# Dylan-H-Wang/skin-sm3

Measured on AMD Instinct MI355X. Metric: SM3 pretrain images/sec (paired 224x224), higher is better.
Workload: dtype bf16

## Files before the change

### skin-sm3_amd/csrc/conv_wgrad.hip

```cpp
#include <stdlib.h>

#include <atomic>

#include "conv_common.h"

namespace {

struct WgradParams {
    const char* x;
    const char* dy;
    float* dw;
    int M, Hi, Wi, Ci, Co;
    int sy, sx, ntaps;
    int dyt[SM3_MAX_TAPS], dxt[SM3_MAX_TAPS], wtap[SM3_MAX_TAPS];
    int w_row_stride;
    int HoWo, Wo, Ho;
    int adv_n, adv_oy, adv_ox;
    FastDiv div_HoWo, div_Wo;
    int tilesCo, tilesCi;
    int k_per_split;
    int gx, splits;
    uint32_t x_bytes;
    const char* dy1;
    float* dw1;
    int Co1, views, Mv, splits_view;
    long dw_view_stride, dw1_view_stride;
    long slab_stride;
    int slab_cap;
    float* dw_direct;
    int pair_rule, rmw;
    long g_x_bytes, g_dy_bytes, g_dw;
    int groups, x_ld, dy_ld;
};

#ifdef SM3_STAMP
__device__ unsigned long long* g_wstamp_buf = nullptr;
__device__ long g_wstamp_cap = 0;
#define SM3_WSTAMP_NOW() __builtin_amdgcn_s_memtime()
#endif

using sm3conv::dma16;
using sm3conv::dma_drain;
using sm3conv::kOOB;

template <int ROW_BYTES, bool BF16>
__device__ __forceinline__ uint32_t swz_bytes(int row) {
    if constexpr (!BF16) return 0u;
    else if constexpr (ROW_BYTES >= 256) return (uint32_t)(row & 3) << 6;
    else return (uint32_t)((row >> 1) & 1) << 6;
}

template <typename T, int BMW, int BNW, int KP, bool DENSE, int NST, int KG = 1, bool GRP = false>
__global__ __launch_bounds__(256 * KG, NST == 1 ? 4 : 1) void conv_wgrad_kernel(const WgradParams p) {
    static_assert(!GRP || DENSE, "grouped launches: the dense (1x1) loader");
    constexpr int SZ = sizeof(T);
    constexpr bool kBf16 = (SZ == 2);
    constexpr int RA = BMW * SZ, RB = BNW * SZ;
    constexpr int A_BYTES = KP * RA, B_BYTES = KP * RB, STAGE = A_BYTES + B_BYTES;
    constexpr int RPI_A = 1024 / RA, RPI_B = 1024 / RB;
    constexpr int AI = A_BYTES / 4096, BI = B_BYTES / 4096;
    constexpr int WTM = BMW / 2, WTN = BNW / 2, TM = WTM / 32, TN = WTN / 32;
    static_assert(AI >= 1 && BI >= 1 && TM >= 1 && TN >= 1 && RA <= 512 && RB <= 512, "unsupported tile");

    extern __shared__ __attribute__((aligned(16))) char smem[];
    const int tid = threadIdx.x, lane = tid & 63;
    const int wave_all = __builtin_amdgcn_readfirstlane(tid >> 6);
    const int wave = wave_all & 3, grp = wave_all >> 2;
#ifdef SM3_STAMP
    const unsigned long long st_entry = SM3_WSTAMP_NOW(), st_rentry = __builtin_amdgcn_s_memrealtime();
    unsigned long long st_seg[4] = {0, 0, 0, 0}, st_loop0 = 0, st_loop1 = 0;
#endif
    const int wm = wave >> 1, wn = wave & 1;

    int bx, slice;
    if (p.splits >= 8) {
        const int xcd = blockIdx.x & 7, q = blockIdx.x >> 3;
        bx = q % p.gx;
        slice = (q / p.gx) * 8 + xcd;
    } else {
        bx = blockIdx.x % p.gx;
        slice = blockIdx.x / p.gx;
    }
    if (slice >= p.splits) return;
    const int tci = bx % p.tilesCi;
    bx /= p.tilesCi;
    const int tap = bx % p.ntaps;
    const int tco = bx / p.ntaps;
    const int ci0 = tci * BNW;
    const bool second = tco * BMW >= p.Co;
    const int co0 = second ? tco * BMW - p.Co : tco * BMW;
    const int dyC = second ? p.Co1 : p.Co;
    const long gid = GRP ? (long)blockIdx.y : 0;
    const char* const dy_base = (second ? p.dy1 : p.dy) + (GRP ? gid * p.g_dy_bytes : 0);
    const char* const x_base = GRP ? p.x + gid * p.g_x_bytes : p.x;
    const int dyP = GRP ? p.dy_ld : dyC;
    const int xP = GRP ? p.x_ld : p.Ci;
    const int view = slice / p.splits_view;
    const int kbeg0 = view * p.Mv + (slice - view * p.splits_view) * p.k_per_split;
    const int kend = min((view + 1) * p.Mv, kbeg0 + p.k_per_split);
    if (kbeg0 >= kend) return;
    const int nsteps = ((kend - kbeg0 + KP - 1) / KP + KG - 1) / KG;
    const int kbeg = kbeg0 + grp * nsteps * KP;
    const int ddy = p.dyt[tap], ddx = p.dxt[tap];

    const __amdgpu_buffer_rsrc_t rdy =
        __builtin_amdgcn_make_buffer_rsrc((void*)dy_base, 0, (uint32_t)kend * (uint32_t)(dyP * SZ), 0x00020000);
    const __amdgpu_buffer_rsrc_t rx = __builtin_amdgcn_make_buffer_rsrc(
        (void*)x_base, 0, DENSE ? (uint32_t)kend * (uint32_t)(xP * SZ) : p.x_bytes, 0x00020000);

    const int a_rin = (lane * 16) / RA, a_pos = ((lane * 16) % RA) / 16;
    const int b_rin = (lane * 16) / RB, b_pos = ((lane * 16) % RB) / 16;
    uint32_t a_off[AI], b_off[BI];
    int b_row[BI];
    uint32_t b_cho[BI];
#pragma unroll
    for (int i = 0; i < AI; ++i) {
        const int r = (wave + 4 * i) * RPI_A + a_rin;
        const uint32_t lchunk = ((uint32_t)a_pos * 16u) ^ swz_bytes<RA, kBf16>(r);
        const bool col_ok = co0 + (int)(lchunk / SZ) < dyC;
        a_off[i] = col_ok ? (uint32_t)(kbeg + r) * (uint32_t)(dyP * SZ) + (uint32_t)(co0 * SZ) + lchunk : kOOB;
    }
#pragma unroll
    for (int i = 0; i < BI; ++i) {
        const int r = (wave + 4 * i) * RPI_B + b_rin;
        const uint32_t lchunk = ((uint32_t)b_pos * 16u) ^ swz_bytes<RB, kBf16>(r);
        const bool col_ok = ci0 + (int)(lchunk / SZ) < p.Ci;
        b_row[i] = col_ok ? r : -(1 << 28);
        b_cho[i] = (uint32_t)(ci0 * SZ) + lchunk;
        b_off[i] = col_ok ? (uint32_t)(kbeg + r) * (uint32_t)(xP * SZ) + b_cho[i] : kOOB;
    }
    const uint32_t smem_lds = (uint32_t)(uintptr_t)((__attribute__((address_space(3))) char*)smem);
    int g_m[BI], g_n[BI], g_oy[BI], g_ox[BI];
#pragma unroll
    for (int i = 0; i < BI; ++i) {
        g_m[i] = kbeg + b_row[i];
        const int m = g_m[i] < 0 ? 0 : g_m[i];
        g_n[i] = fdiv(m, p.div_HoWo);
        const int rem = m - g_n[i] * p.HoWo;
        g_oy[i] = fdiv(rem, p.div_Wo);
        g_ox[i] = rem - g_oy[i] * p.Wo;
    }

    auto dma_stage = [&](int stage, int step) {
        const uint32_t sA = smem_lds + (uint32_t)((grp * NST + stage) * STAGE) + (uint32_t)wave * 1024u;
        const uint32_t sB = sA + A_BYTES;
        const uint32_t soff_a = (uint32_t)(step * KP) * (uint32_t)(dyP * SZ);
#pragma unroll
        for (int i = 0; i < AI; ++i) dma16(rdy, sA + i * 4096, a_off[i], soff_a);
        if constexpr (DENSE) {
            const uint32_t soff_b = (uint32_t)(step * KP) * (uint32_t)(xP * SZ);
#pragma unroll
            for (int i = 0; i < BI; ++i) dma16(rx, sB + i * 4096, b_off[i], soff_b);
        } else {
#pragma unroll
            for (int i = 0; i < BI; ++i) {
                uint32_t off = kOOB;
                if (g_m[i] >= 0 && g_m[i] < kend) {
                    const int iy = g_oy[i] * p.sy + ddy, ix = g_ox[i] * p.sx + ddx;
                    if ((unsigned)iy < (unsigned)p.Hi && (unsigned)ix < (unsigned)p.Wi)
                        off = (uint32_t)((g_n[i] * p.Hi + iy) * p.Wi + ix) * (uint32_t)(p.Ci * SZ) + b_cho[i];
                }
                dma16(rx, sB + i * 4096, off, 0u);
                g_m[i] += KP;
                g_n[i] += p.adv_n;
                g_oy[i] += p.adv_oy;
                g_ox[i] += p.adv_ox;
                if (g_ox[i] >= p.Wo) {
                    g_ox[i] -= p.Wo;
                    ++g_oy[i];
                }
                if (g_oy[i] >= p.Ho) {
                    g_oy[i] -= p.Ho;
                    ++g_n[i];
                }
            }
        }
    };

    f32x16 acc[TM][TN];
#pragma unroll
    for (int i = 0; i < TM; ++i)
#pragma unroll
        for (int j = 0; j < TN; ++j)
#pragma unroll
            for (int r = 0; r < 16; ++r) acc[i][j][r] = 0.f;

    uint32_t ra_off[TM], rb_off[TN];
    if constexpr (kBf16) {
        const int g = lane >> 4, ii = lane & 15, q = ii >> 2, pq = ii & 3, h = g >> 1;
        const int colsel = 16 * (g & 1) + 4 * pq;
        const int krow0 = 8 * h + q;
#pragma unroll
        for (int i = 0; i < TM; ++i)
            ra_off[i] = (uint32_t)krow0 * RA + (((uint32_t)(wm * WTM + i * 32 + colsel) * 2u) ^ swz_bytes<RA, true>(q));
#pragma unroll
        for (int j = 0; j < TN; ++j)
            rb_off[j] = A_BYTES + (uint32_t)krow0 * RB + (((uint32_t)(wn * WTN + j * 32 + colsel) * 2u) ^ swz_bytes<RB, true>(q));
    } else {
        const int r = lane & 31, h = lane >> 5;
#pragma unroll
        for (int i = 0; i < TM; ++i) ra_off[i] = (uint32_t)h * RA + (uint32_t)(wm * WTM + i * 32 + r) * 4u;
#pragma unroll
        for (int j = 0; j < TN; ++j) rb_off[j] = A_BYTES + (uint32_t)h * RB + (uint32_t)(wn * WTN + j * 32 + r) * 4u;
    }

    constexpr int PER = AI + BI;
    static_assert(NST >= 1 && NST <= 4 && 2 * PER <= 63, "vmcnt immediates below cover NST <= 4");
    for (int s = 0; s < NST - 1 && s < nsteps; ++s) dma_stage(s, s);
#ifdef SM3_STAMP
    st_loop0 = SM3_WSTAMP_NOW();
#endif

    for (int s = 0; s < nsteps; ++s) {
#ifdef SM3_STAMP
        const unsigned long long q0 = SM3_WSTAMP_NOW();
        unsigned long long q1 = q0, q2 = q0, q3 = q0;
#endif
        if constexpr (NST == 1) {
            if (s > 0) __syncthreads();
            dma_stage(0, s);
            dma_drain();
            __syncthreads();
        } else {
            const int younger = min(NST - 2, nsteps - 1 - s);
            if (younger >= 2) asm volatile("s_waitcnt vmcnt(%0)" ::"n"(2 * PER) : "memory");
            else if (younger == 1) asm volatile("s_waitcnt vmcnt(%0)" ::"n"(PER) : "memory");
            else dma_drain();
#ifdef SM3_STAMP
            q1 = SM3_WSTAMP_NOW();
#endif
            __syncthreads();
#ifdef SM3_STAMP
            q2 = SM3_WSTAMP_NOW();
#endif
            if (s + NST - 1 < nsteps) dma_stage((s + NST - 1) % NST, s + NST - 1);
        }
#ifdef SM3_STAMP
        q3 = SM3_WSTAMP_NOW();
#endif
        const char* sS = smem + (grp * NST + s % NST) * STAGE;
        if constexpr (kBf16) {
#pragma unroll
            for (int ks = 0; ks < KP / 16; ++ks) {
                uint4 fa[TM], fb[TN];
#pragma unroll
                for (int i = 0; i < TM; ++i) {
                    const char* a0 = sS + ra_off[i] + ks * 16 * RA;
                    s16x4 lo = __builtin_amdgcn_ds_read_tr16_b64_v4i16((__attribute__((address_space(3))) s16x4*)(a0));
                    s16x4 hi = __builtin_amdgcn_ds_read_tr16_b64_v4i16(
                        (__attribute__((address_space(3))) s16x4*)(a0 + 4 * RA));
                    uint2 l2 = __builtin_bit_cast(uint2, lo), h2 = __builtin_bit_cast(uint2, hi);
                    fa[i] = make_uint4(l2.x, l2.y, h2.x, h2.y);
                }
#pragma unroll
                for (int j = 0; j < TN; ++j) {
                    const char* b0 = sS + rb_off[j] + ks * 16 * RB;
                    s16x4 lo = __builtin_amdgcn_ds_read_tr16_b64_v4i16((__attribute__((address_space(3))) s16x4*)(b0));
                    s16x4 hi = __builtin_amdgcn_ds_read_tr16_b64_v4i16(
                        (__attribute__((address_space(3))) s16x4*)(b0 + 4 * RB));
                    uint2 l2 = __builtin_bit_cast(uint2, lo), h2 = __builtin_bit_cast(uint2, hi);
                    fb[j] = make_uint4(l2.x, l2.y, h2.x, h2.y);
                }
#pragma unroll
                for (int i = 0; i < TM; ++i)
#pragma unroll
                    for (int j = 0; j < TN; ++j)
                        sm3conv::mma_frag<T>(fa[i], fb[j], acc[i][j]);
            }
        } else {
#pragma unroll 4
            for (int ks = 0; ks < KP / 2; ++ks) {
                float fa[TM], fb[TN];
#pragma unroll
                for (int i = 0; i < TM; ++i) fa[i] = *reinterpret_cast<const float*>(sS + ra_off[i] + ks * 2 * RA);
#pragma unroll
                for (int j = 0; j < TN; ++j) fb[j] = *reinterpret_cast<const float*>(sS + rb_off[j] + ks * 2 * RB);
#pragma unroll
                for (int i = 0; i < TM; ++i)
#pragma unroll
                    for (int j = 0; j < TN; ++j)
                        acc[i][j] = __builtin_amdgcn_mfma_f32_32x32x2f32(fa[i], fb[j], acc[i][j], 0, 0, 0);
            }
        }
#ifdef SM3_STAMP
        const unsigned long long q4 = SM3_WSTAMP_NOW();
        st_seg[0] += q1 - q0; st_seg[1] += q2 - q1; st_seg[2] += q3 - q2; st_seg[3] += q4 - q3;
#endif
    }
#ifdef SM3_STAMP
    st_loop1 = SM3_WSTAMP_NOW();
    struct WStampOut {
        unsigned long long e, re, l0, l1, *seg; int ns, grp, wave;
        __device__ ~WStampOut() {
            const long w = (long)blockIdx.x * (blockDim.x / 64) + (threadIdx.x >> 6);
            if ((threadIdx.x & 63) == 0 && g_wstamp_buf && w < g_wstamp_cap) {
                unsigned long long* o = g_wstamp_buf + w * 16;
                o[0] = e; o[1] = l0; o[2] = l1; o[3] = __builtin_amdgcn_s_memtime();
                o[4] = seg[0]; o[5] = seg[1]; o[6] = seg[2]; o[7] = seg[3];
                o[8] = (unsigned long long)ns; o[9] = blockIdx.x; o[10] = re; o[11] = __builtin_amdgcn_s_memrealtime();
                o[12] = (unsigned long long)grp; o[13] = (unsigned long long)wave;
            }
        }
    } st_out{st_entry, st_rentry, st_loop0, st_loop1, st_seg, nsteps, grp, wave};
#endif

    if constexpr (KG == 2) {
        static_assert(KG * NST * STAGE >= BMW * BNW * 4, "group 1's tile must fit the workgroup's LDS");
        __syncthreads();
        float* xch = reinterpret_cast<float*>(smem + (NST * STAGE >= BMW * BNW * 4 ? NST * STAGE : 0));
        if (grp == 1) {
#pragma unroll
            for (int i = 0; i < TM; ++i)
#pragma unroll
                for (int j = 0; j < TN; ++j)
#pragma unroll
                    for (int r = 0; r < 16; ++r) xch[((wave * TM * TN + i * TN + j) * 16 + r) * 64 + lane] = acc[i][j][r];
        }
        __syncthreads();
        if (grp == 1) return;
#pragma unroll
        for (int i = 0; i < TM; ++i)
#pragma unroll
            for (int j = 0; j < TN; ++j)
#pragma unroll
                for (int r = 0; r < 16; ++r) acc[i][j][r] += xch[((wave * TM * TN + i * TN + j) * 16 + r) * 64 + lane];
    }
    const int frow = lane & 31, fh = lane >> 5;
    float* const dw_out = (p.slab_stride ? p.dw + (long)slice * p.slab_stride
                           : second    ? p.dw1 + (long)view * p.dw1_view_stride
                                       : p.dw + (long)view * p.dw_view_stride) + (GRP ? gid * p.g_dw : 0);
#pragma unroll
    for (int i = 0; i < TM; ++i)
#pragma unroll
        for (int j = 0; j < TN; ++j)
#pragma unroll
            for (int r = 0; r < 16; ++r) {
                const int co = co0 + wm * WTM + i * 32 + (r & 3) + 8 * (r >> 2) + 4 * fh;
                const int ci = ci0 + wn * WTN + j * 32 + frow;
                const long kcol = (long)p.wtap[tap] * p.Ci + ci;
                if (co < dyC && ci < p.Ci && kcol < p.w_row_stride) {
                    if (p.slab_stride) dw_out[(long)co * p.w_row_stride + kcol] = acc[i][j][r];
                    else if (p.rmw) dw_out[(long)co * p.w_row_stride + kcol] += acc[i][j][r];
                    else atomicAdd(dw_out + (long)co * p.w_row_stride + kcol, acc[i][j][r]);
                }
            }
}

struct Wgrad9Params {
    const char* x;
    const char* dy;
    float* dw;
    int H, W, Ci, Co, R, RW;
    int kblocks, XR;
    int spi;
    int stages_view, stages_per_split, splits_view, splits, gx, tilesCi;
    int wcol[9];
    int w_row_stride;
    uint32_t x_bytes, dy_bytes;
    long slab_stride, dw_view_stride;
    int rmw;
    int img_view;
};

template <typename T, int NST, int KB>
__global__ __launch_bounds__(256, 2) void conv_wgrad9_kernel(const Wgrad9Params p) {
    static_assert(sizeof(T) == 2 && (NST == 1 || NST == 2), "16-bit types, one or two stages");
    const int kblocks = KB ? KB : p.kblocks;
    constexpr int ROWB = 128;
    extern __shared__ __attribute__((aligned(16))) char smem[];
    const int tid = threadIdx.x, lane = tid & 63;
    const int wave = __builtin_amdgcn_readfirstlane(tid >> 6);
    const int wm = wave >> 1, wn = wave & 1;

    int bx, slice;
    if (p.splits >= 8) {
        const int xcd = blockIdx.x & 7, q = blockIdx.x >> 3;
        bx = q % p.gx;
        slice = (q / p.gx) * 8 + xcd;
    } else {
        bx = blockIdx.x % p.gx;
        slice = blockIdx.x / p.gx;
    }
    if (slice >= p.splits) return;
// ... 65 lines not shown
    for (int s = 0; s < nst; ++s) {
        if constexpr (NST == 1) {
            if (s > 0) __syncthreads();
            dma_stage(0, stage0 + s);
            dma_drain();
            __syncthreads();
        } else {
            dma_drain();
            __syncthreads();
            if (s + 1 < nst) dma_stage((s + 1) & 1, stage0 + s + 1);
        }
        const char* sA = smem + (NST == 2 ? (s & 1) * STAGE : 0);
        const char* sB = sA + A_BYTES;
        auto kblock = [&](int ks) {
            const char* a0 = sA + ra_off + ks * 16 * ROWB;
            const s16x4 alo = __builtin_amdgcn_ds_read_tr16_b64_v4i16((__attribute__((address_space(3))) s16x4*)(a0));
            const s16x4 ahi = __builtin_amdgcn_ds_read_tr16_b64_v4i16((__attribute__((address_space(3))) s16x4*)(a0 + 4 * ROWB));
            const uint4 mm = *reinterpret_cast<const uint4*>(smem + m_off + ks * 64);
            const uint4 mp = *reinterpret_cast<const uint4*>(smem + m_off + ks * 64 + 16);
            const uint2 l2 = __builtin_bit_cast(uint2, alo), h2 = __builtin_bit_cast(uint2, ahi);
            uint4 fa[3];
            fa[1] = make_uint4(l2.x, l2.y, h2.x, h2.y);
            fa[0] = make_uint4(l2.x & mm.x, l2.y & mm.y, h2.x & mm.z, h2.y & mm.w);
            fa[2] = make_uint4(l2.x & mp.x, l2.y & mp.y, h2.x & mp.z, h2.y & mp.w);
#pragma unroll
            for (int t = 0; t < 9; ++t) {
                const char* b0 = sB + rb_off[t] + ks * 16 * ROWB;
                const s16x4 lo = __builtin_amdgcn_ds_read_tr16_b64_v4i16((__attribute__((address_space(3))) s16x4*)(b0));
                const s16x4 hi = __builtin_amdgcn_ds_read_tr16_b64_v4i16((__attribute__((address_space(3))) s16x4*)(b0 + 4 * ROWB));
                const uint2 bl = __builtin_bit_cast(uint2, lo), bh = __builtin_bit_cast(uint2, hi);
                const uint4 fb = make_uint4(bl.x, bl.y, bh.x, bh.y);
                sm3conv::mma_frag<T>(fa[t % 3], fb, acc[t]);
            }
        };
        if constexpr (KB > 0) {
#pragma unroll
            for (int ks = 0; ks < KB; ++ks) kblock(ks);
        } else {
#pragma unroll 1
            for (int ks = 0; ks < kblocks; ++ks) kblock(ks);
        }
    }

    const int frow = lane & 31, fh = lane >> 5;
    float* const dw_out = p.slab_stride ? p.dw + (long)slice * p.slab_stride : p.dw + (long)view * p.dw_view_stride;
    float* const o0 = dw_out + (long)(co0 + wm * 32 + 4 * fh) * p.w_row_stride + ci0 + wn * 32 + frow;
    auto emit = [&](auto&& put) {
#pragma unroll
        for (int t = 0; t < 9; ++t)
#pragma unroll
            for (int r = 0; r < 16; ++r) put(o0 + (long)((r & 3) + 8 * (r >> 2)) * p.w_row_stride + p.wcol[t], acc[t][r]);
    };
    if (p.slab_stride) emit([](float* o, float v) { *o = v; });
    else if (p.rmw) emit([](float* o, float v) { *o += v; });
    else emit([](float* o, float v) { atomicAdd(o, v); });
}

static thread_local int g_last_slabs = 0;

static int env_int(const char* name, int dflt) {
    const char* v = getenv(name);
    return v ? atoi(v) : dflt;
}

static int current_device() {
    int dev = 0;
    if (hipGetDevice(&dev) != hipSuccess || dev < 0 || dev > 31) dev = 0;
    return dev;
}

static int cus_per_xcd() {
    static std::atomic<int> v{0};
    int r = v.load(std::memory_order_relaxed);
    if (!r) {
        int cus = 0;
        if (hipDeviceGetAttribute(&cus, hipDeviceAttributeMultiprocessorCount, current_device()) != hipSuccess || cus < 8)
            cus = 256;
        r = cus / 8;
        v.store(r, std::memory_order_relaxed);
    }
    return r;
}

template <typename T, int BMW, int BNW, int KP, bool DENSE, int NST, int KG = 1, bool GRP = false>
int launch_wgrad_kp(WgradParams p, hipStream_t st) {
    constexpr int SZ = sizeof(T);
    constexpr int LDS = KG * NST * KP * (BMW * SZ + BNW * SZ);
    if (p.Co1 > 0 && p.Co % BMW) return SM3_EALIGN;
    p.tilesCo = (p.Co + BMW - 1) / BMW + (p.Co1 + BMW - 1) / BMW;
    p.tilesCi = (p.Ci + BNW - 1) / BNW;
    p.adv_n = KP / p.HoWo;
    p.adv_oy = (KP % p.HoWo) / p.Wo;
    p.adv_ox = (KP % p.HoWo) % p.Wo;
    const long gx = (long)p.tilesCo * p.ntaps * p.tilesCi;
    auto kern = conv_wgrad_kernel<T, BMW, BNW, KP, DENSE, NST, KG, GRP>;
    static std::atomic<int> per_cu_dev[32];
    const int dev = current_device();
    int per_cu = per_cu_dev[dev].load(std::memory_order_acquire);
    if (!per_cu) {
        if (LDS > 65536) {
            hipError_t e = hipFuncSetAttribute(reinterpret_cast<const void*>(kern),
                                               hipFuncAttributeMaxDynamicSharedMemorySize, LDS);
            if (e != hipSuccess) return (int)e;
        }
        int n = 0;
        if (hipOccupancyMaxActiveBlocksPerMultiprocessor(&n, kern, 256 * KG, LDS) != hipSuccess || n < 1) n = 1;
        per_cu = n;
        per_cu_dev[dev].store(n, std::memory_order_release);
    }
    const long slots_xcd = (long)cus_per_xcd() * per_cu;
    const long target = env_int("SM3_WGRAD_TARGET_CTAS", 0);
    long splits;
    if (target > 0) splits = (target + gx - 1) / gx;
    else if (gx <= slots_xcd) splits = 8 * (slots_xcd / gx);
    else splits = 8 * slots_xcd / gx;
    splits = (p.slab_stride && p.pair_rule) ? (splits + 1) / 2 : (splits + p.views - 1) / p.views;
    if (p.slab_stride && splits > p.slab_cap) splits = p.slab_cap;
    const long max_splits = (p.Mv + KP * 8 * KG - 1) / (KP * 8 * KG);
    if (splits > max_splits) splits = max_splits;
    if (splits < 1) splits = 1;
    long kps = (p.Mv + splits - 1) / splits;
    kps = (kps + KP - 1) / KP * KP;
    splits = (p.Mv + kps - 1) / kps;
    p.k_per_split = (int)kps;
    p.gx = (int)gx;
    p.splits_view = (int)splits;
    g_last_slabs = (int)splits;
    splits *= p.views;
    p.splits = (int)splits;
    if (p.slab_stride && p.dw_direct && splits == 1) {
        p.slab_stride = 0;
        p.rmw = 1;
        p.dw = p.dw_direct;
        g_last_slabs = 0;
    }
    const long nblocks = gx * (splits >= 8 ? (splits + 7) / 8 * 8 : splits);
    if (gx > 0x7fffffffL || nblocks > 0x7fffffffL) return SM3_EINVAL;
    hipLaunchKernelGGL(kern, dim3((unsigned)nblocks, GRP ? (unsigned)p.groups : 1u), dim3(256 * KG), LDS, st, p);
    SM3_CHECK_LAUNCH();
    return 0;
}

template <typename T, int BMW, int BNW>
int launch_wgrad(WgradParams p, hipStream_t st) {
    constexpr int KP = sizeof(T) == 2 ? 32 : 16;
    const bool dense = p.ntaps == 1 && p.sy == 1 && p.sx == 1 && p.dyt[0] == 0 && p.dxt[0] == 0 &&
                       p.HoWo == p.Hi * p.Wi;
    if (dense) return launch_wgrad_kp<T, BMW, BNW, KP, true, 4, 2>(p, st);
    if constexpr (sizeof(T) == 2) {
        if (p.Ci >= 128) return launch_wgrad_kp<T, BMW, BNW, 64, false, 1>(p, st);
    }
    return launch_wgrad_kp<T, BMW, BNW, KP, false, 2>(p, st);
}

template <typename T>
int launch_wgrad9(const sm3_conv_desc* d, const void* x, const void* dy, float* dw, int views, long dw_view_stride,
                  int slab_cap, float* dw_direct, hipStream_t st) {
    if (!env_int("SM3_WGRAD9", 1)) return 1;
    if (d->ntaps != 9 || d->sy != 1 || d->sx != 1 || d->Hi != d->Ho || d->Wi != d->Wo) return 1;
    if (d->Co % 64 || d->Ci % 64 || d->N % views) return 1;
    for (int t = 0; t < 9; ++t)
        if (d->dy[t] != t / 3 - 1 || d->dx[t] != t % 3 - 1 || d->wtap[t] < 0 || (d->wtap[t] + 1) * d->Ci > d->w_row_stride)
            return 1;
    const int H = d->Ho, W = d->Wo;
    const int force_r = env_int("SM3_WGRAD9_R", 0), force_nst = env_int("SM3_WGRAD9_NST", 0);
    int R = 0, kblocks = 0, XR = 0, nstg = 0;
    long best_num = 0, best_den = 1;
    for (int r = H; r >= 1; --r) {
        if (H % r || (force_r && r != force_r)) continue;
        const int kb = (r * W + 15) / 16, xr = (16 * kb + 2 * W + 2 + 7) / 8 * 8;
        const long stage = (long)(16 * kb + xr) * 128;
        if (kb > 13) continue;
        const int n = force_nst ? force_nst : (2 * stage + kb * 64 <= 81920 ? 2 : stage + kb * 64 <= 81920 ? 1 : 0);
        if (!n || n * stage + kb * 64 > 160 * 1024) continue;
        const long num = (long)r * W, den = 16L * kb;
        const bool better = !R || num * best_den > best_num * den || (num * best_den == best_num * den && n > nstg);
        if (better) { R = r; kblocks = kb; XR = xr; nstg = n; best_num = num; best_den = den; }
    }
    if (R && !force_r && best_num * 100 < best_den * 85) return 1;
    if (!R) return 1;
    Wgrad9Params p;
    p.x = (const char*)x; p.dy = (const char*)dy; p.dw = dw;
    p.H = H; p.W = W; p.Ci = d->Ci; p.Co = d->Co; p.R = R; p.RW = R * W; p.kblocks = kblocks; p.XR = XR;
    p.spi = H / R;
    p.img_view = d->N / views;
    p.stages_view = p.img_view * p.spi;
    p.tilesCi = d->Ci / 64;
    p.gx = (d->Co / 64) * p.tilesCi;
    for (int t = 0; t < 9; ++t) p.wcol[t] = d->wtap[t] * d->Ci;
// ... 53 lines not shown

static int wgrad_impl(const sm3_conv_desc* d, const void* x, const void* dy, float* dw, const void* dy1, int Co1,
                      float* dw1, int views, long dw_view_stride, long dw1_view_stride, void* stream, int slab_cap = 0,
                      float* dw_direct = nullptr) {
    if (!d || !x || !dy || !dw) return SM3_EINVAL;
    if (!SM3_DTYPE_OK(d->dtype)) return SM3_EDTYPE;
    const int sz = d->dtype == SM3_F32 ? 4 : 2;
    if (d->N <= 0 || d->Hi <= 0 || d->Wi <= 0 || d->Ci <= 0 || d->Ho <= 0 || d->Wo <= 0 || d->Co <= 0) return SM3_EINVAL;
    if (d->ntaps < 1 || d->ntaps > SM3_MAX_TAPS) return SM3_EINVAL;
    if ((d->Ci * sz) % 16 != 0 || (d->Co * sz) % 16 != 0 || (Co1 * sz) % 16 != 0) return SM3_EALIGN;
    if (d->osy != 1 || d->osx != 1 || d->ooy != 0 || d->oox != 0 || d->Hout != d->Ho || d->Wout != d->Wo)
        return SM3_EINVAL;
    const long M = (long)d->N * d->Ho * d->Wo;
    if (M > 0x7fffffffL || (long)d->N * d->Hi * d->Wi > 0x7fffffffL) return SM3_EINVAL;
    if (views < 1 || M % views || Co1 < 0 || (Co1 > 0 && (!dy1 || !dw1))) return SM3_EINVAL;
    WgradParams p;
    p.x = (const char*)x; p.dy = (const char*)dy; p.dw = dw;
    p.dy1 = (const char*)dy1; p.dw1 = dw1; p.Co1 = Co1;
    p.views = views; p.Mv = (int)(M / views);
    p.dw_view_stride = dw_view_stride; p.dw1_view_stride = dw1_view_stride;
    p.slab_cap = slab_cap;
    p.slab_stride = slab_cap > 0 ? (long)d->Co * d->w_row_stride : 0;
    p.dw_direct = dw_direct;
    p.pair_rule = dw_direct ? 0 : 1;
    p.rmw = 0;
    p.M = (int)M; p.Hi = d->Hi; p.Wi = d->Wi; p.Ci = d->Ci; p.Co = d->Co;
    p.sy = d->sy; p.sx = d->sx; p.ntaps = d->ntaps;
    for (int t = 0; t < SM3_MAX_TAPS; ++t) { p.dyt[t] = d->dy[t]; p.dxt[t] = d->dx[t]; p.wtap[t] = d->wtap[t]; }
    p.w_row_stride = d->w_row_stride;
    p.HoWo = d->Ho * d->Wo; p.Wo = d->Wo; p.Ho = d->Ho;
    p.div_HoWo = make_fastdiv((uint32_t)p.HoWo);
    p.div_Wo = make_fastdiv((uint32_t)p.Wo);
    const long xb = (long)d->N * d->Hi * d->Wi * d->Ci * sz, yb = M * d->Co * sz, y1b = M * Co1 * sz;
    if (xb >= 0xC0000000L || yb >= 0xC0000000L || y1b >= 0xC0000000L) return SM3_EINVAL;
    p.x_bytes = (uint32_t)xb;
    hipStream_t st = (hipStream_t)stream;
    if (d->dtype != SM3_F32 && Co1 == 0) {
        const int rc = d->dtype == SM3_BF16
                           ? launch_wgrad9<bf16_t>(d, x, dy, dw, views, dw_view_stride, slab_cap, dw_direct, st)
                           : launch_wgrad9<f16_t>(d, x, dy, dw, views, dw_view_stride, slab_cap, dw_direct, st);
        if (rc != 1) return rc;
    }
    const bool nco = d->Co + Co1 <= 64, nci = d->Ci <= 64;
    if (d->dtype == SM3_BF16) {
        if (nco && nci) return launch_wgrad<bf16_t, 64, 64>(p, st);
        if (nco) return launch_wgrad<bf16_t, 64, 128>(p, st);
        if (nci) return launch_wgrad<bf16_t, 128, 64>(p, st);
        return launch_wgrad<bf16_t, 128, 128>(p, st);
    }
    if (d->dtype == SM3_F16) {
        if (nco && nci) return launch_wgrad<f16_t, 64, 64>(p, st);
        if (nco) return launch_wgrad<f16_t, 64, 128>(p, st);
        if (nci) return launch_wgrad<f16_t, 128, 64>(p, st);
        return launch_wgrad<f16_t, 128, 128>(p, st);
    }
    if (nco && nci) return launch_wgrad<float, 64, 64>(p, st);
    if (nco) return launch_wgrad<float, 64, 128>(p, st);
    if (nci) return launch_wgrad<float, 128, 64>(p, st);
    return launch_wgrad<float, 128, 128>(p, st);
}

#ifdef SM3_STAMP
extern "C" int sm3_debug_set_wgrad_stamps(void* buf, long capacity_waves) {
    unsigned long long* b = (unsigned long long*)buf;
    if (hipMemcpyToSymbol(HIP_SYMBOL(g_wstamp_buf), &b, sizeof(b)) != hipSuccess) return SM3_EINVAL;
    if (hipMemcpyToSymbol(HIP_SYMBOL(g_wstamp_cap), &capacity_waves, sizeof(long)) != hipSuccess) return SM3_EINVAL;
    return 0;
}
#endif

extern "C" int sm3_conv_wgrad(const sm3_conv_desc* d, const void* x, const void* dy, float* dw, void* stream) {
    return wgrad_impl(d, x, dy, dw, nullptr, 0, nullptr, 1, 0, 0, stream);
}

extern "C" int sm3_conv_wgrad_slabs(const sm3_conv_desc* d, const void* x, const void* dy, float* slabs, int slab_capacity,
                                    int views, int* slabs_used, void* stream) {
    if (!slabs_used || slab_capacity < 1) return SM3_EINVAL;
    if (d && d->ntaps * d->Ci != d->w_row_stride) return SM3_EINVAL;
    const int rc = wgrad_impl(d, x, dy, slabs, nullptr, 0, nullptr, views, 0, 0, stream, slab_capacity);
    if (rc == 0) *slabs_used = g_last_slabs;
    return rc;
}

__global__ __launch_bounds__(256) void slab_reduce_kernel(const float* __restrict__ slabs, int nslabs, long n,
                                                          float* __restrict__ out, int accumulate) {
    __shared__ float4 red[8][32];
    const int col = threadIdx.x & 31, jl = threadIdx.x >> 5;
    const long e4 = ((long)blockIdx.x * 32 + col) * 4;
    float4 a0 = make_float4(0.f, 0.f, 0.f, 0.f), a1 = a0, a2 = a0, a3 = a0;
    auto add = [](float4& a, const float4& b) { a.x += b.x; a.y += b.y; a.z += b.z; a.w += b.w; };
    if (e4 < n) {
        const float* src = slabs + e4;
        int j = jl;
        for (; j + 24 < nslabs; j += 32) {
            const float4 v0 = *reinterpret_cast<const float4*>(src + (long)j * n);
            const float4 v1 = *reinterpret_cast<const float4*>(src + (long)(j + 8) * n);
            const float4 v2 = *reinterpret_cast<const float4*>(src + (long)(j + 16) * n);
            const float4 v3 = *reinterpret_cast<const float4*>(src + (long)(j + 24) * n);
            add(a0, v0); add(a1, v1); add(a2, v2); add(a3, v3);
        }
        for (; j < nslabs; j += 8) add(a0, *reinterpret_cast<const float4*>(src + (long)j * n));
        add(a0, a1);
        add(a2, a3);
        add(a0, a2);
    }
    red[jl][col] = a0;
    __syncthreads();
    if (jl == 0 && e4 < n) {
        float4 t = red[0][col];
#pragma unroll
        for (int l = 1; l < 8; ++l) add(t, red[l][col]);
        float4* o = reinterpret_cast<float4*>(out + e4);
        if (accumulate) {
            float4 g = *o;
            add(g, t);
            t = g;
        }
        *o = t;
    }
}

extern "C" int sm3_slab_reduce(const float* slabs, int nslabs, int64_t n, float* out, int accumulate, void* stream) {
    if (!slabs || !out || nslabs < 1 || n < 4 || n % 4) return SM3_EINVAL;
    if (((uintptr_t)slabs | (uintptr_t)out) & 15) return SM3_EALIGN;
    const long blocks = (n / 4 + 31) / 32;
    if (blocks > 0x7fffffffL) return SM3_EINVAL;
    hipLaunchKernelGGL(slab_reduce_kernel, dim3((unsigned)blocks), dim3(256), 0, (hipStream_t)stream, slabs, nslabs, (long)n,
                       out, accumulate);
    SM3_CHECK_LAUNCH();
    return 0;
}

extern "C" int sm3_conv_wgrad_det(const sm3_conv_desc* d, const void* x, const void* dy, float* dw, float* slabs,
                                  int slab_capacity, void* stream) {
    if (!slabs || !dw || slab_capacity < 1) return SM3_EINVAL;
    if (d && d->ntaps * d->Ci != d->w_row_stride) return SM3_EINVAL;
    if (((uintptr_t)slabs | (uintptr_t)dw) & 15) return SM3_EALIGN;
    const int rc = wgrad_impl(d, x, dy, slabs, nullptr, 0, nullptr, 1, 0, 0, stream, slab_capacity, dw);
    if (rc != 0 || g_last_slabs == 0) return rc;
    return sm3_slab_reduce(slabs, g_last_slabs, (int64_t)d->Co * d->w_row_stride, dw, 1, stream);
}

extern "C" int sm3_conv_wgrad_cat(const sm3_conv_desc* d, const void* x, const void* dy, float* dw, const void* dy1,
                                  int Co1, float* dw1, int views, int64_t dw_view_stride, int64_t dw1_view_stride,
                                  void* stream) {
    if (Co1 > 0 && d && d->Co % 128) return SM3_EALIGN;
    return wgrad_impl(d, x, dy, dw, dy1, Co1, dw1, views, (long)dw_view_stride, (long)dw1_view_stride, stream);
}

extern "C" int sm3_grouped_wgrad_det(int dtype, const void* x, const void* dy, float* dw, float* slabs, int slab_capacity,
                                     int rows, int groups, int K, int N, void* stream) {
    if (dtype != SM3_F32) return SM3_EDTYPE;
    if (!x || !dy || !dw || !slabs || slab_capacity < 1 || rows <= 0 || groups <= 0 || groups > 65535 || K <= 0 || N <= 0)
        return SM3_EINVAL;
    if ((K * 4) % 16 != 0 || (N * 4) % 16 != 0) return SM3_EALIGN;
    if (((uintptr_t)slabs | (uintptr_t)dw) & 15) return SM3_EALIGN;
    if ((long)rows * groups * K * 4 >= 0xC0000000L || (long)rows * groups * N * 4 >= 0xC0000000L) return SM3_EINVAL;
    WgradParams p;
    p.x = (const char*)x; p.dy = (const char*)dy; p.dw = slabs;
    p.dy1 = nullptr; p.dw1 = nullptr; p.Co1 = 0;
    p.views = 1; p.Mv = rows;
    p.dw_view_stride = 0; p.dw1_view_stride = 0;
    p.slab_cap = slab_capacity;
    p.slab_stride = (long)groups * N * K;
    p.dw_direct = dw;
    p.pair_rule = 0;
    p.rmw = 0;
    p.M = rows; p.Hi = 1; p.Wi = 1; p.Ci = K; p.Co = N;
    p.sy = 1; p.sx = 1; p.ntaps = 1;
    for (int t = 0; t < SM3_MAX_TAPS; ++t) { p.dyt[t] = 0; p.dxt[t] = 0; p.wtap[t] = 0; }
    p.w_row_stride = K;
    p.HoWo = 1; p.Wo = 1; p.Ho = 1;
    p.div_HoWo = make_fastdiv(1u);
    p.div_Wo = make_fastdiv(1u);
    p.x_bytes = (uint32_t)((long)rows * groups * K * 4);
    p.groups = groups;
    p.g_x_bytes = (long)K * 4;
    p.g_dy_bytes = (long)N * 4;
    p.g_dw = (long)N * K;
    p.x_ld = groups * K;
    p.dy_ld = groups * N;
    hipStream_t st = (hipStream_t)stream;
    const bool nco = N <= 64, nci = K <= 64;
    int rc;
    if (nco && nci) rc = launch_wgrad_kp<float, 64, 64, 16, true, 4, 2, true>(p, st);
    else if (nco) rc = launch_wgrad_kp<float, 64, 128, 16, true, 4, 2, true>(p, st);
    else if (nci) rc = launch_wgrad_kp<float, 128, 64, 16, true, 4, 2, true>(p, st);
    else rc = launch_wgrad_kp<float, 128, 128, 16, true, 4, 2, true>(p, st);
    if (rc != 0 || g_last_slabs == 0) return rc;
    return sm3_slab_reduce(slabs, g_last_slabs, (int64_t)groups * N * K, dw, 1, stream);
}
```

Measured before the change: 4677.

## Add split slab-reduce kernel for many small slabs and optional wgrad K-group stagger

```diff
diff --git a/scratch/r7_slab_reduce_ab.py b/scratch/r7_slab_reduce_ab.py
--- /dev/null
+++ b/scratch/r7_slab_reduce_ab.py
@@ -0,0 +1,53 @@
+import ctypes as C, os, sys
+sys.path.insert(0, os.path.join(os.path.dirname(os.path.abspath(__file__)), "..", "skin-sm3_amd"))
+import torch
+from sm3hip import _lib, ops
+
+new = _lib.load()
+old = C.CDLL(os.environ["SM3_PARENT_LIBRARY"])
+dev = torch.device("cuda:0")
+
+
+def call(lib, slabs, ns, n, out):
+    rc = lib.sm3_slab_reduce(C.c_void_p(slabs.data_ptr()), C.c_int(ns), C.c_int64(n), C.c_void_p(out.data_ptr()), C.c_int(1),
+                             C.c_void_p(torch.cuda.current_stream().cuda_stream))
+    assert rc == 0, rc
+
+
+def timed(fn, reps=100):
+    fn(); torch.cuda.synchronize()
+    st = torch.cuda.Stream()
+    g = torch.cuda.CUDAGraph()
+    with torch.cuda.stream(st):
+        with torch.cuda.graph(g, stream=st):
+            for _ in range(reps):
+                fn()
+    g.replay(); torch.cuda.synchronize()
+    e0, e1 = torch.cuda.Event(enable_timing=True), torch.cuda.Event(enable_timing=True)
+    e0.record()
+    g.replay()
+    e1.record(); torch.cuda.synchronize()
+    return e0.elapsed_time(e1) / reps * 1e3
+
+
+print(f"{'nslabs x n':28s}{'parent':>10s}{'form1':>10s}{'form2':>10s}{'auto':>10s}")
+for n in (64 * 64, 128 * 128, 256 * 256, 1024 * 256, 2048 * 512):
+    for ns in (8, 16, 32, 64, 128, 256):
+        if ns * n > (1 << 26):
+            continue
+        slabs = torch.randn(ns * n, device=dev)
+        out = torch.zeros(n, device=dev)
+        res = {}
+        for r in range(3):
+            for name, lib, form in (("parent", old, None), ("form1", new, "1"), ("form2", new, "2"), ("auto", new, "0")):
+                if form is not None:
+                    os.environ["SM3_SLAB_REDUCE_FORM"] = form
+                res[name] = min(res.get(name, 1e30), timed(lambda: call(lib, slabs, ns, n, out)))
+        o = []
+        for name, lib, form in (("parent", old, None), ("form1", new, "1"), ("form2", new, "2")):
+            if form is not None:
+                os.environ["SM3_SLAB_REDUCE_FORM"] = form
+            out.zero_(); call(lib, slabs, ns, n, out); o.append(out.clone())
+        same = torch.equal(o[0], o[1]) and torch.equal(o[0], o[2])
+        print(f"{ns:4d} x {n:9d}            " + "".join(f"{res[k]:10.1f}" for k in ("parent", "form1", "form2", "auto")) +
+              f"   bits {'equal' if same else 'DIFFER'}", flush=True)
diff --git a/scratch/r7_wgrad_stagger_ab.py b/scratch/r7_wgrad_stagger_ab.py
--- /dev/null
+++ b/scratch/r7_wgrad_stagger_ab.py
@@ -0,0 +1,72 @@
+import os, sys
+sys.path.insert(0, os.path.join(os.path.dirname(os.path.abspath(__file__)), "..", "skin-sm3_amd"))
+import torch
+from sm3hip import ops
+
+dt = torch.bfloat16
+code = ops.dtype_code(dt)
+dev = torch.device("cuda:0")
+SHAPES = [(512, 56, 64, 256, 1), (512, 14, 256, 1024, 1), (512, 28, 128, 512, 1), (512, 14, 1024, 256, 0), (512, 56, 256, 64, 0),
+          (512, 28, 512, 128, 0), (512, 7, 512, 2048, 1), (512, 56, 256, 128, 0), (512, 56, 64, 64, 1), (512, 28, 512, 256, 0),
+          (512, 14, 256, 256, 1), (512, 7, 2048, 512, 0), (512, 28, 256, 512, 1), (256, 1, 2048, 2048, 0), (512, 14, 1024, 512, 0),
+          (512, 7, 1024, 2048, 1), (512, 14, 512, 1024, 1), (512, 28, 128, 128, 1), (512, 56, 64, 64, 0), (512, 1, 2048, 2048, 0),
+          (512, 7, 512, 512, 1), (512, 28, 256, 256, 1), (512, 7, 1024, 1024, 1), (256, 1, 2048, 128, 0), (512, 14, 512, 512, 1)]
+VARIANTS = [("lockstep", {"SM3_WGRAD_STAGGER": "0"}), ("half", {"SM3_WGRAD_STAGGER": "1"}), ("full", {"SM3_WGRAD_STAGGER": "2"})]
+if os.environ.get("AB_PARENT"):
+    VARIANTS = [("parent", {})]
+
+
+def setenv(env):
+    for k in ("SM3_WGRAD_STAGGER", "SM3_WGRAD_STAGGER_RING"):
+        os.environ.pop(k, None)
+    os.environ.update(env)
+
+
+def timed(fn, reps):
+    fn()
+    torch.cuda.synchronize()
+    e0, e1 = torch.cuda.Event(enable_timing=True), torch.cuda.Event(enable_timing=True)
+    e0.record()
+    for _ in range(reps):
+        fn()
+    e1.record()
+    torch.cuda.synchronize()
+    return e0.elapsed_time(e1) / reps * 1e3
+
+
+tot = {n: 0.0 for n, _ in VARIANTS}
+print(f"{'shape':44s}" + "".join(f"{n:>12s}" for n, _ in VARIANTS) + "   (us per call, min of 5 rounds x 10; slab form: launch only)")
+for N, H, Ci, Co, slabform in SHAPES:
+    M = N * H * H
+    x = torch.randn(M, Ci, device=dev).to(dt)
+    dy = torch.randn(M, Co, device=dev).to(dt)
+    d = ops.fwd_desc(code, N, H, H, Ci, Co, 1, 1, 0)
+    n = Co * Ci
+    if slabform:
+        cap = min(ops.SLAB_CAP, ops.wgrad_det_cap(n))
+        slabs = torch.empty(2 * cap * n, device=dev)
+        fn = lambda: ops.conv_wgrad_slabs(d, x, dy, slabs, views=2, cap=cap)
+    else:
+        cap = ops.wgrad_det_cap(n)
+        slabs = torch.empty(cap * n, device=dev)
+        dw = torch.zeros(Co, Ci, device=dev)
+        fn = lambda: ops.conv_wgrad_det(d, x, dy, dw, slabs, cap)
+    outs = {}
+    best = {name: 1e30 for name, _ in VARIANTS}
+    for r in range(5):
+        for name, env in VARIANTS:
+            setenv(env)
+            best[name] = min(best[name], timed(fn, 10))
+    for name, env in VARIANTS:
+        setenv(env)
+        if slabform:
+            slabs.zero_(); used = fn(); outs[name] = slabs[: 2 * used * n].clone()
+        else:
+            dw.zero_(); fn(); outs[name] = dw.clone()
+    same = all(torch.equal(outs[VARIANTS[0][0]], o) for o in outs.values())
+    tag = f"M{M}_K1x{Ci}_N{Co}" + ("_v2_slabs" if slabform else "")
+    print(f"{tag:44s}" + "".join(f"{best[nm]:12.1f}" for nm, _ in VARIANTS) + f"   bits {'equal' if same else 'DIFFER'}", flush=True)
+    for nm, _ in VARIANTS:
+        tot[nm] += best[nm]
+    del x, dy, slabs
+print(f"{'sum (one call each)':44s}" + "".join(f"{tot[nm]:12.1f}" for nm, _ in VARIANTS))
diff --git a/skin-sm3_amd/csrc/conv_wgrad.hip b/skin-sm3_amd/csrc/conv_wgrad.hip
--- a/skin-sm3_amd/csrc/conv_wgrad.hip
+++ b/skin-sm3_amd/csrc/conv_wgrad.hip
@@ -1,6 +1,7 @@
 #include <stdlib.h>
 
 #include <atomic>
+#include <type_traits>
 
 #include "conv_common.h"
 
@@ -31,6 +32,7 @@
     int pair_rule, rmw;
     long g_x_bytes, g_dy_bytes, g_dw;
     int groups, x_ld, dy_ld;
+    int stagger;
 };
 
 #ifdef SM3_STAMP
@@ -50,9 +52,10 @@
     else return (uint32_t)((row >> 1) & 1) << 6;
 }
 
-template <typename T, int BMW, int BNW, int KP, bool DENSE, int NST, int KG = 1, bool GRP = false>
+template <typename T, int BMW, int BNW, int KP, bool DENSE, int NST, int KG = 1, bool GRP = false, bool STG = false>
 __global__ __launch_bounds__(256 * KG, NST == 1 ? 4 : 1) void conv_wgrad_kernel(const WgradParams p) {
     static_assert(!GRP || DENSE, "grouped launches: the dense (1x1) loader");
+    static_assert(!STG || (KG == 2 && NST > 1), "the stagger is between the two K-groups of a ring");
     constexpr int SZ = sizeof(T);
     constexpr bool kBf16 = (SZ == 2);
     constexpr int RA = BMW * SZ, RB = BNW * SZ;
@@ -68,7 +71,7 @@
     const int wave = wave_all & 3, grp = wave_all >> 2;
 #ifdef SM3_STAMP
     const unsigned long long st_entry = SM3_WSTAMP_NOW(), st_rentry = __builtin_amdgcn_s_memrealtime();
-    unsigned long long st_seg[4] = {0, 0, 0, 0}, st_loop0 = 0, st_loop1 = 0;
+    unsigned long long st_seg[5] = {0, 0, 0, 0, 0}, st_loop0 = 0, st_loop1 = 0;
 #endif
     const int wm = wave >> 1, wn = wave & 1;
 
@@ -206,15 +209,63 @@
 
     constexpr int PER = AI + BI;
     static_assert(NST >= 1 && NST <= 4 && 2 * PER <= 63, "vmcnt immediates below cover NST <= 4");
+    constexpr bool kStag = STG;
+    const int stag = kStag && grp == 1 ? p.stagger : 0;
     for (int s = 0; s < NST - 1 && s < nsteps; ++s) dma_stage(s, s);
 #ifdef SM3_STAMP
     st_loop0 = SM3_WSTAMP_NOW();
 #endif
 
+    struct Frag {
+        std::conditional_t<kBf16, uint4, float> a[TM], b[TN];
+    };
+    auto load_frag = [&](const char* sS, int ks, Frag& f) {
+        if constexpr (kBf16) {
+#pragma unroll
+            for (int i = 0; i < TM; ++i) {
+                const char* a0 = sS + ra_off[i] + ks * 16 * RA;
+                s16x4 lo = __builtin_amdgcn_ds_read_tr16_b64_v4i16((__attribute__((address_space(3))) s16x4*)(a0));
+                s16x4 hi = __builtin_amdgcn_ds_read_tr16_b64_v4i16((__attribute__((address_space(3))) s16x4*)(a0 + 4 * RA));
+                uint2 l2 = __builtin_bit_cast(uint2, lo), h2 = __builtin_bit_cast(uint2, hi);
+                f.a[i] = make_uint4(l2.x, l2.y, h2.x, h2.y);
+            }
+#pragma unroll
+            for (int j = 0; j < TN; ++j) {
+                const char* b0 = sS + rb_off[j] + ks * 16 * RB;
+                s16x4 lo = __builtin_amdgcn_ds_read_tr16_b64_v4i16((__attribute__((address_space(3))) s16x4*)(b0));
+                s16x4 hi = __builtin_amdgcn_ds_read_tr16_b64_v4i16((__attribute__((address_space(3))) s16x4*)(b0 + 4 * RB));
+                uint2 l2 = __builtin_bit_cast(uint2, lo), h2 = __builtin_bit_cast(uint2, hi);
+                f.b[j] = make_uint4(l2.x, l2.y, h2.x, h2.y);
+            }
+        } else {
+#pragma unroll
+            for (int i = 0; i < TM; ++i) f.a[i] = *reinterpret_cast<const float*>(sS + ra_off[i] + ks * 2 * RA);
+#pragma unroll
+            for (int j = 0; j < TN; ++j) f.b[j] = *reinterpret_cast<const float*>(sS + rb_off[j] + ks * 2 * RB);
+        }
+    };
+    auto mma = [&](const Frag& f) {
+#pragma unroll
+        for (int i = 0; i < TM; ++i)
+#pragma unroll
+            for (int j = 0; j < TN; ++j) {
+                if constexpr (kBf16) sm3conv::mma_frag<T>(f.a[i], f.b[j], acc[i][j]);
+                else acc[i][j] = __builtin_amdgcn_mfma_f32_32x32x2f32(f.a[i], f.b[j], acc[i][j], 0, 0, 0);
+            }
+    };
+    constexpr int KB = kBf16 ? KP / 16 : KP / 2;
+    static_assert(!kStag || KB % 2 == 0, "a staggered stage has two halves");
+    constexpr int UNR = kBf16 ? KB : 4;
+    Frag held[kStag ? KB : 1];
+    auto mma_half = [&](int h) {
+#pragma unroll
+        for (int ks = 0; ks < KB / 2; ++ks) mma(held[h ? ks + KB / 2 : ks]);
+    };
+
     for (int s = 0; s < nsteps; ++s) {
 #ifdef SM3_STAMP
         const unsigned long long q0 = SM3_WSTAMP_NOW();
-        unsigned long long q1 = q0, q2 = q0, q3 = q0;
+        unsigned long long q1 = q0, q2 = q0, q3 = q0, q4 = q0;
 #endif
         if constexpr (NST == 1) {
             if (s > 0) __syncthreads();
@@ -226,6 +277,9 @@
             if (younger >= 2) asm volatile("s_waitcnt vmcnt(%0)" ::"n"(2 * PER) : "memory");
             else if (younger == 1) asm volatile("s_waitcnt vmcnt(%0)" ::"n"(PER) : "memory");
             else dma_drain();
+            if constexpr (kStag) {
+                if (stag) asm volatile("s_waitcnt lgkmcnt(0)" ::: "memory");
+            }
 #ifdef SM3_STAMP
             q1 = SM3_WSTAMP_NOW();
 #endif
@@ -233,59 +287,60 @@
 #ifdef SM3_STAMP
             q2 = SM3_WSTAMP_NOW();
 #endif
+        }
+        const char* sS = smem + (grp * NST + s % NST) * STAGE;
+        if constexpr (kStag) {
+            if (stag && s > 0) {
+                if (stag == 2) mma_half(0);
+                mma_half(1);
+            }
+#ifdef SM3_STAMP
+            q3 = SM3_WSTAMP_NOW();
+#endif
             if (s + NST - 1 < nsteps) dma_stage((s + NST - 1) % NST, s + NST - 1);
-        }
-#ifdef SM3_STAMP
-        q3 = SM3_WSTAMP_NOW();
-#endif
-        const char* sS = smem + (grp * NST + s % NST) * STAGE;
-        if constexpr (kBf16) {
-#pragma unroll
-            for (int ks = 0; ks < KP / 16; ++ks) {
-                uint4 fa[TM], fb[TN];
-#pragma unroll
-                for (int i = 0; i < TM; ++i) {
-                    const char* a0 = sS + ra_off[i] + ks * 16 * RA;
-                    s16x4 lo = __builtin_amdgcn_ds_read_tr16_b64_v4i16((__attribute__((address_space(3))) s16x4*)(a0));
-                    s16x4 hi = __builtin_amdgcn_ds_read_tr16_b64_v4i16(
-                        (__attribute__((address_space(3))) s16x4*)(a0 + 4 * RA));
-                    uint2 l2 = __builtin_bit_cast(uint2, lo), h2 = __builtin_bit_cast(uint2, hi);
-                    fa[i] = make_uint4(l2.x, l2.y, h2.x, h2.y);
-                }
-#pragma unroll
-                for (int j = 0; j < TN; ++j) {
-                    const char* b0 = sS + rb_off[j] + ks * 16 * RB;
-                    s16x4 lo = __builtin_amdgcn_ds_read_tr16_b64_v4i16((__attribute__((address_space(3))) s16x4*)(b0));
-                    s16x4 hi = __builtin_amdgcn_ds_read_tr16_b64_v4i16(
-                        (__attribute__((address_space(3))) s16x4*)(b0 + 4 * RB));
-                    uint2 l2 = __builtin_bit_cast(uint2, lo), h2 = __builtin_bit_cast(uint2, hi);
-                    fb[j] = make_uint4(l2.x, l2.y, h2.x, h2.y);
-                }
-#pragma unroll
-                for (int i = 0; i < TM; ++i)
-#pragma unroll
-                    for (int j = 0; j < TN; ++j)
-                        sm3conv::mma_frag<T>(fa[i], fb[j], acc[i][j]);
-            }
+#ifdef SM3_STAMP
+            q4 = SM3_WSTAMP_NOW();
+#endif
+#pragma unroll
+            for (int ks = 0; ks < KB; ++ks) load_frag(sS, ks, held[ks]);
+            if (stag != 2) {
+                mma_half(0);
+                if (stag == 0) mma_half(1);
+            }
+#ifdef SM3_STAMP
+            const unsigned long long q5 = SM3_WSTAMP_NOW();
+            st_seg[0] += q1 - q0; st_seg[1] += q2 - q1; st_seg[2] += q4 - q3; st_seg[3] += q5 - q4; st_seg[4] += q3 - q2;
+#endif
         } else {
-#pragma unroll 4
-            for (int ks = 0; ks < KP / 2; ++ks) {
-                float fa[TM], fb[TN];
-#pragma unroll
-                for (int i = 0; i < TM; ++i) fa[i] = *reinterpret_cast<const float*>(sS + ra_off[i] + ks * 2 * RA);
-#pragma unroll
-                for (int j = 0; j < TN; ++j) fb[j] = *reinterpret_cast<const float*>(sS + rb_off[j] + ks * 2 * RB);
-#pragma unroll
-                for (int i = 0; i < TM; ++i)
-#pragma unroll
-                    for (int j = 0; j < TN; ++j)
-                        acc[i][j] = __builtin_amdgcn_mfma_f32_32x32x2f32(fa[i], fb[j], acc[i][j], 0, 0, 0);
-            }
-        }
-#ifdef SM3_STAMP
-        const unsigned long long q4 = SM3_WSTAMP_NOW();
-        st_seg[0] += q1 - q0; st_seg[1] += q2 - q1; st_seg[2] += q3 - q2; st_seg[3] += q4 - q3;
-#endif
+            if constexpr (NST > 1) {
+                if (s + NST - 1 < nsteps) dma_stage((s + NST - 1) % NST, s + NST - 1);
+            }
+#ifdef SM3_STAMP
+            q3 = SM3_WSTAMP_NOW();
+#endif
+#pragma unroll UNR
+            for (int ks = 0; ks < KB; ++ks) {
+                Frag f;
+                load_frag(sS, ks, f);
+                mma(f);
+            }
+#ifdef SM3_STAMP
+            q4 = SM3_WSTAMP_NOW();
+            st_seg[0] += q1 - q0; st_seg[1] += q2 - q1; st_seg[2] += q3 - q2; st_seg[3] += q4 - q3;
+#endif
+        }
+    }
+    if constexpr (kStag) {
+        if (stag) {
+#ifdef SM3_STAMP
+            const unsigned long long q0 = SM3_WSTAMP_NOW();
+#endif
+            if (stag == 2) mma_half(0);
+            mma_half(1);
+#ifdef SM3_STAMP
+            st_seg[4] += SM3_WSTAMP_NOW() - q0;
+#endif
+        }
     }
 #ifdef SM3_STAMP
     st_loop1 = SM3_WSTAMP_NOW();
@@ -298,7 +353,7 @@
                 o[0] = e; o[1] = l0; o[2] = l1; o[3] = __builtin_amdgcn_s_memtime();
                 o[4] = seg[0]; o[5] = seg[1]; o[6] = seg[2]; o[7] = seg[3];
                 o[8] = (unsigned long long)ns; o[9] = blockIdx.x; o[10] = re; o[11] = __builtin_amdgcn_s_memrealtime();
-                o[12] = (unsigned long long)grp; o[13] = (unsigned long long)wave;
+                o[12] = (unsigned long long)grp; o[13] = (unsigned long long)wave; o[14] = seg[4];
             }
         }
     } st_out{st_entry, st_rentry, st_loop0, st_loop1, st_seg, nsteps, grp, wave};
@@ -530,10 +585,18 @@
     return r;
 }
 
-template <typename T, int BMW, int BNW, int KP, bool DENSE, int NST, int KG = 1, bool GRP = false>
+template <typename T, int BMW, int BNW, int KP, bool DENSE, int NST, int KG = 1, bool GRP = false, bool STG = false>
 int launch_wgrad_kp(WgradParams p, hipStream_t st) {
     constexpr int SZ = sizeof(T);
     constexpr int LDS = KG * NST * KP * (BMW * SZ + BNW * SZ);
+    if constexpr (KG == 2 && NST > 1 && !STG) {
+        const int v = env_int("SM3_WGRAD_STAGGER", 0);
+        if (v == 1 || v == 2) {
+            p.stagger = v;
+            return launch_wgrad_kp<T, BMW, BNW, KP, DENSE, NST, KG, GRP, true>(p, st);
+        }
+    }
+    if constexpr (!STG) p.stagger = 0;
     if (p.Co1 > 0 && p.Co % BMW) return SM3_EALIGN;
     p.tilesCo = (p.Co + BMW - 1) / BMW + (p.Co1 + BMW - 1) / BMW;
     p.tilesCi = (p.Ci + BNW - 1) / BNW;
@@ -541,7 +604,7 @@
     p.adv_oy = (KP % p.HoWo) / p.Wo;
     p.adv_ox = (KP % p.HoWo) % p.Wo;
     const long gx = (long)p.tilesCo * p.ntaps * p.tilesCi;
-    auto kern = conv_wgrad_kernel<T, BMW, BNW, KP, DENSE, NST, KG, GRP>;
+    auto kern = conv_wgrad_kernel<T, BMW, BNW, KP, DENSE, NST, KG, GRP, STG>;
     static std::atomic<int> per_cu_dev[32];
     const int dev = current_device();
     int per_cu = per_cu_dev[dev].load(std::memory_order_acquire);
@@ -551,8 +614,14 @@
                                                hipFuncAttributeMaxDynamicSharedMemorySize, LDS);
             if (e != hipSuccess) return (int)e;
         }
+        auto kern_rule = conv_wgrad_kernel<T, BMW, BNW, KP, DENSE, NST, KG, GRP, false>;
+        if (STG && LDS > 65536) {
+            hipError_t e = hipFuncSetAttribute(reinterpret_cast<const void*>(kern_rule),
+                                               hipFuncAttributeMaxDynamicSharedMemorySize, LDS);
+            if (e != hipSuccess) return (int)e;
+        }
         int n = 0;
-        if (hipOccupancyMaxActiveBlocksPerMultiprocessor(&n, kern, 256 * KG, LDS) != hipSuccess || n < 1) n = 1;
+        if (hipOccupancyMaxActiveBlocksPerMultiprocessor(&n, kern_rule, 256 * KG, LDS) != hipSuccess || n < 1) n = 1;
         per_cu = n;
         per_cu_dev[dev].store(n, std::memory_order_release);
     }
@@ -772,38 +841,78 @@
     return rc;
 }
 
+__device__ __forceinline__ void slab_add(float4& a, const float4& b) { a.x += b.x; a.y += b.y; a.z += b.z; a.w += b.w; }
+
 __global__ __launch_bounds__(256) void slab_reduce_kernel(const float* __restrict__ slabs, int nslabs, long n,
                                                           float* __restrict__ out, int accumulate) {
     __shared__ float4 red[8][32];
     const int col = threadIdx.x & 31, jl = threadIdx.x >> 5;
     const long e4 = ((long)blockIdx.x * 32 + col) * 4;
     float4 a0 = make_float4(0.f, 0.f, 0.f, 0.f), a1 = a0, a2 = a0, a3 = a0;
-    auto add = [](float4& a, const float4& b) { a.x += b.x; a.y += b.y; a.z += b.z; a.w += b.w; };
     if (e4 < n) {
         const float* src = slabs + e4;
+        auto ld = [&](int j) { return *reinterpret_cast<const float4*>(src + (long)j * n); };
         int j = jl;
         for (; j + 24 < nslabs; j += 32) {
-            const float4 v0 = *reinterpret_cast<const float4*>(src + (long)j * n);
-            const float4 v1 = *reinterpret_cast<const float4*>(src + (long)(j + 8) * n);
-            const float4 v2 = *reinterpret_cast<const float4*>(src + (long)(j + 16) * n);
-            const float4 v3 = *reinterpret_cast<const float4*>(src + (long)(j + 24) * n);
-            add(a0, v0); add(a1, v1); add(a2, v2); add(a3, v3);
-        }
-        for (; j < nslabs; j += 8) add(a0, *reinterpret_cast<const float4*>(src + (long)j * n));
-        add(a0, a1);
-        add(a2, a3);
-        add(a0, a2);
+            const float4 v0 = ld(j), v1 = ld(j + 8), v2 = ld(j + 16), v3 = ld(j + 24);
+            slab_add(a0, v0); slab_add(a1, v1); slab_add(a2, v2); slab_add(a3, v3);
+        }
+        for (; j < nslabs; j += 8) slab_add(a0, ld(j));
+        slab_add(a0, a1);
+        slab_add(a2, a3);
+        slab_add(a0, a2);
     }
     red[jl][col] = a0;
     __syncthreads();
     if (jl == 0 && e4 < n) {
         float4 t = red[0][col];
 #pragma unroll
-        for (int l = 1; l < 8; ++l) add(t, red[l][col]);
+        for (int l = 1; l < 8; ++l) slab_add(t, red[l][col]);
         float4* o = reinterpret_cast<float4*>(out + e4);
         if (accumulate) {
             float4 g = *o;
-            add(g, t);
+            slab_add(g, t);
+            t = g;
+        }
+        *o = t;
+    }
+}
+
+__global__ __launch_bounds__(256) void slab_reduce_split_kernel(const float* __restrict__ slabs, int nslabs, long n,
+                                                                float* __restrict__ out, int accumulate) {
+    __shared__ float4 red[8][4][8];
+    const int col = threadIdx.x & 7, q = (threadIdx.x >> 3) & 3, jl = threadIdx.x >> 5;
+    const long e4 = ((long)blockIdx.x * 8 + col) * 4;
+    float4 a = make_float4(0.f, 0.f, 0.f, 0.f);
+    if (e4 < n) {
+        const float* src = slabs + e4;
+        auto ld = [&](int j) { return *reinterpret_cast<const float4*>(src + (long)j * n); };
+        int j = jl;
+        for (; j + 24 + 96 < nslabs; j += 128) {
+            const float4 v0 = ld(j + 8 * q), v1 = ld(j + 8 * q + 32), v2 = ld(j + 8 * q + 64), v3 = ld(j + 8 * q + 96);
+            slab_add(a, v0); slab_add(a, v1); slab_add(a, v2); slab_add(a, v3);
+        }
+        for (; j + 24 < nslabs; j += 32) slab_add(a, ld(j + 8 * q));
+        if (q == 0)
+            for (; j < nslabs; j += 8) slab_add(a, ld(j));
+    }
+    red[jl][q][col] = a;
+    __syncthreads();
+    if (threadIdx.x < 8 && e4 < n) {
+        float4 t;
+#pragma unroll
+        for (int l = 0; l < 8; ++l) {
+            float4 s0 = red[l][0][col], s2 = red[l][2][col];
+            slab_add(s0, red[l][1][col]);
+            slab_add(s2, red[l][3][col]);
+            slab_add(s0, s2);
+            if (l == 0) t = s0;
+            else slab_add(t, s0);
+        }
+        float4* o = reinterpret_cast<float4*>(out + e4);
+        if (accumulate) {
+            float4 g = *o;
+            slab_add(g, t);
             t = g;
         }
         *o = t;
@@ -813,10 +922,12 @@
 extern "C" int sm3_slab_reduce(const float* slabs, int nslabs, int64_t n, float* out, int accumulate, void* stream) {
     if (!slabs || !out || nslabs < 1 || n < 4 || n % 4) return SM3_EINVAL;
     if (((uintptr_t)slabs | (uintptr_t)out) & 15) return SM3_EALIGN;
-    const long blocks = (n / 4 + 31) / 32;
+    const int form = env_int("SM3_SLAB_REDUCE_FORM", 0);
+    const bool split = form ? form == 2 : (nslabs >= 128 && n <= 16384);
+    const long blocks = split ? (n / 4 + 7) / 8 : (n / 4 + 31) / 32;
     if (blocks > 0x7fffffffL) return SM3_EINVAL;
-    hipLaunchKernelGGL(slab_reduce_kernel, dim3((unsigned)blocks), dim3(256), 0, (hipStream_t)stream, slabs, nslabs, (long)n,
-                       out, accumulate);
+    hipLaunchKernelGGL(split ? slab_reduce_split_kernel : slab_reduce_kernel, dim3((unsigned)blocks), dim3(256), 0,
+                       (hipStream_t)stream, slabs, nslabs, (long)n, out, accumulate);
     SM3_CHECK_LAUNCH();
     return 0;
 }
```

Result: no change. 4679, median of 4 (+0.1%).
